# zhaoyizhou1123/OfflineRL-Kit

Measured on AMD Instinct MI355X. Metric: gradient-steps/sec (CQL, batch=256), higher is better.
Workload: dtype f32 storage / accumulate; products on split-fp16 MFMA (every operand = fp16 hi + fp16 lo plane = 22 significand bits, power-of-two operand scales folded back into the fp32 accumulators, hi*hi + hi*lo + lo*hi on v_mfma_f32_16x16x32_f16; the reference's fp32 has 24): losses and Q-values meet the 1e-4

## Files before the change

offlinerl-kit_amd/csrc/engine.h:

```cpp
#pragma once
#include <hip/hip_runtime.h>

#include <map>
#include <set>
#include <string>
#include <vector>

#include "../../include/orl_engine.h"
#include "gemm.h"
#include "kernels.h"
#include "ws_gemm.h"
#include "small_fwd.h"
#include "small_bwd.h"

namespace orl {

void set_error(const std::string& msg);
int fail(const std::string& msg);
#define ORL_HIP(expr)                                                                            \
  do {                                                                                           \
    hipError_t _e = (expr);                                                                      \
    if (_e != hipSuccess) {                                                                      \
      ::orl::set_error(std::string(#expr) + ": " + hipGetErrorString(_e));                       \
      return -1;                                                                                 \
// ... 205 lines not shown
    prof_begin(p3 ? (std::string(tag) + "@p3").c_str() : tag, flops, bytes);
    const hipError_t err = launch();
    prof_end();
    return err == hipSuccess ? 0 : fail(std::string(what) + " launch " + tag + ": " + hipGetErrorString(err));
  }
  int tail_add(const ZOut& out, long out_sm, const ZOut& part, int nparts, int M, int nz1, const char* tag);
  WsFwdP ws_fwd_p(const Mat& X, int M, const NetRef& nr, int layer, const Mat& Y, const Mat* dmask) const;
  int ws_dgrad(const DY& dy, int M, const NetRef& nr, int layer, const Mat& maskH, const Mat* w0_X, const Mat* dX, int max_blocks, const char* tag, int* slabs);
  int ws_wgrad(const DY& dy, const Mat& X, int M, const NetRef& nr, int layer, const Mat* recompute_X0, const char* tag, int* slabs);
  SmallFwdP small_fwd_p(const Mat& X, int M, const NetRef& nr, const Mat* H0, const Mat* H1, const Mat& out) const;
  int linear_fwd(const Mat& X, int M, const NetRef& nr, int layer, const Mat& Y, int epi, const Mat* maskH, const char* tag,
                 int in_row0 = 0, int in_rows = -1, const Mat* tail_out = nullptr, bool* tail_fused = nullptr,
                 const Mat* fuse_X0 = nullptr, const char* tag0 = nullptr, const float* x_dscale = nullptr);
  int tq_scratch_nets = 2;
  int linear_dgrad(const DY& dy, int M, const NetRef& nr, int layer, int col0, int ncols, const Mat* maskH, const Mat& dX, const char* tag,
                   const Mat* w0_X = nullptr, bool store_dx = true, int* w0_slabs = nullptr);
  int linear_wgrad(const DY& dy, const Mat& X, int M, const NetRef& nr, int layer, int ksplit, int slab0, bool with_bias,
                   const char* tag, int in_row0 = 0, int in_rows = -1, bool* fuse_tail = nullptr, int* slabs_out = nullptr,
                   const float* x_dscale = nullptr, const Mat* recompute_X0 = nullptr);
  bool recompute_h0 = false;
  bool recompute_h0_ok(const NetLayout& l, int layer, int M, int nz) const {
    return recompute_h0 && layer == 1 && l.L >= 3 && !l.ens && ws_precision_ok() && ws_wgrad_rows_ok(M, nz);
  }
  int adam(int net, int nnets, int lr_slot, const std::vector<std::pair<long, int>>& segs, int target_net, unsigned long long t_div = 1);
  int polyak(int target_net, int src_net, int nnets);
  void prof_begin(const char* name, double flops, double bytes = 0);
  void prof_end();
  int assemble(const Mat& obs, const Mat* act, const Mat& X, int row0, int rows, int rep);
  int mlp_forward(const Mat& X, int M, const NetRef& nr, std::vector<Mat>& hs, const Mat& out, const char* tag,
                  const SampleJob* jobs = nullptr, int njobs = 0, bool* jobs_done = nullptr);
  int mlp_qgrad(const Mat& X, int M, const NetRef& nr, const Mat& q, const Mat& G, int gc0, int gn, const char* tag, bool* done);
  int mlp_forward_only(const Mat& X, int M, const NetRef& nr, std::vector<Mat>& hs, const Mat& out, const char* tag,
                       const SampleJob* jobs = nullptr, int njobs = 0, bool* jobs_done = nullptr);
  bool fwd_only = false;
  int mlp_forward_dropout(const Mat& X, int M, const NetRef& nr, std::vector<Mat>& hs, const Mat& out, const char* tag, float p,
                          const std::vector<Mat>& masks);
  int scale_inplace(const Mat& m, int rows, int cols, int nets, float s, const Mat* mask, const char* tag);
  bool no_ws = false;
  float bwd_scale = 1.0f;

  int enqueue_sample();
  int enqueue_noise();
  int enqueue_step(int variant);
  int step_variant() const;
  int n_variants() const;
  int build_common();
// ... 12 lines not shown
```

offlinerl-kit_amd/csrc/engine.hip:

```cpp
#include "engine.h"

#include <math.h>
#include <stdio.h>
#include <stdlib.h>
#include <string.h>

#include <algorithm>
#include <tuple>

namespace orl {

static thread_local std::string g_err;
void set_error(const std::string& msg) { g_err = msg; }
int fail(const std::string& msg) {
  set_error(msg);
  return -1;
}

static inline int rup(int x, int m) { return (x + m - 1) / m * m; }

static void add_tensor(NetLayout& l, const std::string& name, long off, std::initializer_list<long> shape) {
  TensorInfo t;
  t.name = name;
  t.off = off;
// ... 431 lines not shown
    }
  }
  const int nz = R * nr.nz1;
  int cfg = pick_cfg(p.M, p.N, p.K, nz);
  if (cfg == CFG_SQ) cfg = CFG_SQ8;
  if (epi == E_BIAS_RELU && ws_precision_ok() && !no_ws && !force_scalar && in_row0 == 0 && in_rows == in &&
      Y.bits && Y.pitch == out && (long)M * nz >= ws_fwd_min_rows) {
    WsFwdP w = ws_fwd_p(X, M, nr, layer, Y, nullptr);
    const bool want_tail = tail_out && tail_fused && layer == l.L - 1 && l.out_dim == 1;
    if (want_tail) { w.tw = nr.w(l.L); w.tb = nr.b(l.L); w.tq = tail_out->zo(); w.tq_sm = tail_out->pitch; }
    const bool elide = want_tail && layer >= 1 && (fwd_only || (elide_top && !l.ens && ws_wgrad_rows_ok(M, nz)));
    if (elide) w.Y.p = nullptr;
    const bool ws_ok = ws_fwd_supported(w, in, out);
    bool fused0 = false;
    if (ws_ok && fuse_X0 && layer == 1 && X.bits && X.pitch == in) {
      w.X0 = fuse_X0->z(); w.x0_pitch = fuse_X0->pitch; w.in0 = l.layer_in(0);
      w.W0 = nr.w(0);
      if (l.ens) { w.w0_sn = 1; w.w0_sk = l.layer_out(0); } else { w.w0_sn = l.layer_in(0); w.w0_sk = 1; }
      w.b0 = nr.b(0);
      w.mb0 = X.zbits(); w.mb0_g = X.bg;
      fused0 = ws_fwd01_supported(w) && aligned16(fuse_X0->p);
      if (!fused0) w.X0.p = nullptr;
      else if (fwd_only || (!want_tail && recompute_h0_ok(l, layer, M, nz))) w.x0_discard = 1;
    }
    if (fuse_X0 && !fused0) {
      if (linear_fwd(*fuse_X0, M, nr, 0, X, E_BIAS_RELU, nullptr, tag0 ? tag0 : tag)) return -1;
      fuse_X0 = nullptr;
    }
    if (ws_ok) {
      bool fwd3 = false;
      if (p3(1) && (fused0 || !w.X0.p) && ws_dump && (!want_tail || ws.count("tq_scratch"))) {
        bool room = true;
        if (want_tail) {
          const Mat& sc = ws.at("tq_scratch");
          room = (long)M <= sc.cs && nr.nz1 <= tq_scratch_nets;
          if (room) w.tq2 = sc.zo();
        }
        if (room) {
          w.np3 = 1; w.dump = ws_dump;
          fwd3 = ws_fwd3_supported(w, in, out);
          if (!fwd3) { w.np3 = 0; w.tq2.p = nullptr; w.dump = nullptr; }
        }
      }
      const double f0 = fused0 ? 2.0 * M * (double)in * (w.in0 + 1) * nz : 0.0;
      if (fused0) bits_live.insert(X.bits);
      if (w.x0_discard) vals_dead.insert(X.p);
// ... 87 lines not shown
  GemmP p;
  memset(&p, 0, sizeof(p));
  p.a_dscale = cur_gscale; p.b_scale = ORL_WSCALE;
  if (mm_prec() == P_SPLIT3) p.a_scale = ORL_GSCALE3;
  p.A = dy.m.z();
  p.a_sr = dy.m.pitch; p.a_sk = 1;
  if (dy.rank1) {
    p.a_trans = 0;
    p.rowv = dy.rowv.z();
    p.colv = nr.w(l.L);
  }
  p.B = nr.w(layer);
  if (l.ens) { p.B.p += (long)col0 * out; p.b_sr = out; p.b_sk = 1; }
  else { p.B.p += col0; p.b_sr = 1; p.b_sk = in; p.b_rlim = (in - col0) & ~3; }
  p.C = dX.p; p.c_s0 = dX.rs; p.c_s1 = dX.cs; p.c_sr = dX.pitch; p.c_sn = 1;
  p.M = M; p.N = ncols; p.K = out;
  p.nz1 = nr.nz1; p.ksplit = 1;
  if (maskH) { p.aux = maskH->z(); p.aux_sr = maskH->pitch; }
  const int nz = R * nr.nz1;
  if (w0_slabs) *w0_slabs = 0;
  if (maskH && maskH->bits && bits_live.count(maskH->bits) && ncols == maskH->pitch && aligned16(maskH->p) && (maskH->pitch & 3) == 0) {
    p.aux_bits = maskH->bits; p.xb_s0 = maskH->brs; p.xb_s1 = maskH->bcs; p.xb_g = maskH->bg;
  }
  if (w0_X && w0_slabs && !store_dx && maskH && dy.rank1 && layer == 1 && col0 == 0 && !l.ens && !force_scalar &&
      ws_precision_ok() && p.aux_bits && dy.m.bits && bits_live.count(dy.m.bits) && out == dy.m.pitch &&
      ncols == in && (long)M * nz >= ws_bwd_min_rows) {
    const int rc = ws_dgrad(dy, M, nr, layer, *maskH, w0_X, nullptr, max_slab, tag, w0_slabs);
    if (rc <= 0) return rc;
  }
  if (!(w0_X && w0_slabs) && maskH && dy.rank1 && col0 == 0 && !force_scalar && ws_precision_ok() && p.aux_bits &&
      dy.m.bits && bits_live.count(dy.m.bits) && out == dy.m.pitch && ncols == in && dX.pitch >= in && (long)M * nz >= ws_bwd_min_rows) {
    const int rc = ws_dgrad(dy, M, nr, layer, *maskH, nullptr, &dX, 1 << 20, tag, nullptr);
    if (rc <= 0) return rc;
  }
  if (w0_X && w0_slabs && !store_dx && maskH && !dy.rank1 && layer == 1 && col0 == 0 && !force_scalar && ws_precision_ok() &&
      p.aux_bits && dy.m.pitch == out && ncols == in && (long)M * nz >= ws_dgrad_plain_min_rows) {
    const int rc = ws_dgrad(dy, M, nr, layer, *maskH, w0_X, nullptr, max_slab, tag, w0_slabs);
    if (rc <= 0) return rc;
  }
  if (w0_X && w0_slabs && maskH && layer == 1 && col0 == 0 && !l.ens && !force_scalar) {
    const int slabs = w0_fused_slabs(p, nz, l.layer_in(0), w0_X->pitch, w0_X->p, w0_X->rs, w0_X->cs, max_slab);
    if (slabs > 0) {
      float* g = grads + nr.g_off;
      p.w0_x = w0_X->z(); p.w0_xsr = w0_X->pitch; p.w0_in = l.layer_in(0);
      p.w0_out = g + l.w_off[0]; p.w0_bias = g + l.b_off[0];
      p.w0_s0 = (long)max_slab * P_train; p.w0_s1 = l.w_ms[0]; p.w0_bs1 = l.b_ms[0]; p.w0_ks = P_train; p.w0_sr = l.layer_in(0);
// ... 47 lines not shown
  if (Krows >= 4096) ks = std::max(ks, wgrad_long_min);
  if (cfg == CFG_SQ && Krows < 1024 && kchunks >= 8) ks = std::max(ks, wgrad_small_ks);
  ks = std::max(1, std::min(ks, std::min(ksplit_cap, kchunks)));
  while (ks > 1 && (kchunks + ks - 1) / ks < 2) --ks;
  return ks;
}

int Engine::ws_wgrad(const DY& dy, const Mat& X, int M, const NetRef& nr, int layer, const Mat* recompute_X0, const char* tag, int* slabs) {
  const NetLayout& l = *nr.lay;
  const int in = l.layer_in(layer), out = l.layer_out(layer), nz = R * nr.nz1;
  const bool derived = dy.rank1 && vals_dead.count(dy.m.p) > 0;
  float* g = grads + nr.g_off;
  WsWgradP w;
  memset(&w, 0, sizeof(w));
  w.H0 = X.z(); w.h0_pitch = X.pitch;
  w.dW = g + l.w_off[layer]; w.db = g + l.b_off[layer];
  w.o_rs = (long)max_slab * P_train; w.o_msw = l.w_ms[layer]; w.o_msb = l.b_ms[layer]; w.o_ks = P_train;
  if (dy.rank1) {
    w.abits = dy.m.zbits(); w.ab_g = dy.m.bg;
    w.dq = dy.rowv.z(); w.dq_sm = dy.rowv.pitch;
    w.wt = nr.w(l.L);
    if (derived) { w.W1 = nr.w(layer); w.b1 = nr.b(layer); }
    else { w.H1 = dy.m.z(); w.h1_pitch = dy.m.pitch; }
    w.dwt = g + l.w_off[l.L]; w.dbt = g + l.b_off[l.L]; w.o_mswt = l.w_ms[l.L]; w.o_msbt = l.b_ms[l.L];
    w.np3 = p3(4) && derived;
    w.lab_clk = lab_clk(72);
  } else {
    w.dZ = dy.m.z(); w.dz_pitch = dy.m.pitch;
    if (recompute_X0) {
      w.X0 = recompute_X0->z(); w.x0_pitch = recompute_X0->pitch; w.in0 = l.layer_in(0);
      w.W0 = nr.w(0); w.w0_sn = l.layer_in(0); w.w0_sk = 1;
      w.b0 = nr.b(0);
    }
  }
  w.M = M; w.nz1 = nr.nz1; w.f32 = ws_f32(); w.gscale = cur_gscale;
  if (!ws_wgrad_supported(w, out, in)) return 1;
  const bool w3 = !dy.rank1 && p3(4) && ws_wgrad3p_supported(w, out, in);
  const int per_z = ws_dgrad_blocks(M, w3 ? 2 * nz : nz, dy.rank1 ? ws_wgrad_slab_cap : max_slab, ws_geo, 1 << 20);
  const double flops = 2.0 * M * (double)in * (dy.rank1 ? out + 2 : out + 1 + (recompute_X0 ? w.in0 + 1 : 0)) * nz;
  const double bytes = dy.rank1 ? nz * ((derived ? M * (double)out / 8 : 4.0 * M * (double)out) + 4.0 * M * (in + 1) + 4.0 * per_z * out * (in + 2))
                                : nz * (4.0 * M * (double)((recompute_X0 ? w.x0_pitch : in) + out) + 4.0 * per_z * out * (in + 1));
  if (timed("ws_wgrad", tag, w3 || w.np3, flops, bytes, [&] { return w3 ? launch_ws_wgrad3p(w, nz, per_z, stream) : launch_ws_wgrad(w, nz, per_z, stream); })) return -1;
  *slabs = per_z;
  return 0;
}

int Engine::linear_wgrad(const DY& dy, const Mat& X, int M, const NetRef& nr, int layer, int ksplit, int slab0, bool with_bias,
                         const char* tag, int in_row0, int in_rows, bool* fuse_tail, int* slabs_out, const float* x_dscale, const Mat* recompute_X0) {
  const NetLayout& l = *nr.lay;
  const int in = l.layer_in(layer), out = l.layer_out(layer);
  if (in_rows < 0) in_rows = in;
  if (slab0 + ksplit > max_slab) return fail("wgrad: slab budget exceeded");
  const bool x_dead = vals_dead.count(X.p) > 0;
  if (x_dead && !(recompute_X0 && layer == 1)) return fail(std::string("wgrad ") + tag + ": the input activation was not stored by the forward pass");
  GemmP p;
  memset(&p, 0, sizeof(p));
  p.a_dscale = cur_gscale; p.b_dscale = x_dscale;
  if (mm_prec() == P_SPLIT3) { p.a_scale = ORL_GSCALE3; if (x_dscale) p.b_scale = ORL_GSCALE3; }
  p.A = dy.m.z();
  p.a_sr = 1; p.a_sk = dy.m.pitch;
  if (out == 1 && dy.m.pitch == 1 && !dy.rank1) p.a_sr = 4;
  if (dy.rank1) {
    p.a_trans = 1;
    p.rowv = dy.rowv.z();
    p.colv = nr.w(l.L);
  }
  p.B = X.z();
  p.b_sr = 1; p.b_sk = X.pitch;
  p.a_rlim = dy.m.pitch & ~3; p.b_rlim = X.pitch & ~3;
  p.ones_row = 1 << 30;
  p.M = out; p.N = in_rows; p.K = M;
  p.nz1 = nr.nz1; p.ksplit = ksplit;
  const long g_rs = (long)max_slab * P_train;
  float* g = grads + nr.g_off + (long)slab0 * P_train;
  if (l.ens) { p.C = g + l.w_off[layer] + (long)in_row0 * out; p.c_sr = 1; p.c_sn = out; }
  else { p.C = g + l.w_off[layer] + in_row0; p.c_sr = in; p.c_sn = 1; }
  p.c_s0 = g_rs; p.c_s1 = l.w_ms[layer]; p.c_ks = P_train;
  if (with_bias) { p.bias_out = g + l.b_off[layer]; p.bo_s0 = g_rs; p.bo_s1 = l.b_ms[layer]; p.bo_ks = P_train; }
  const int nz = R * nr.nz1;
  if (slabs_out) *slabs_out = ksplit;
  if (slabs_out && fuse_tail && dy.rank1 && with_bias && slab0 == 0 && ws_precision_ok() && !force_scalar && !l.ens &&
      dy.m.bits && bits_live.count(dy.m.bits) && out == dy.m.pitch && in_row0 == 0 && in_rows == in && X.pitch == in &&
      ws_wgrad_rows_ok(M, nz)) {
    const int rc = ws_wgrad(dy, X, M, nr, layer, nullptr, tag, slabs_out);
    if (rc == 0) *fuse_tail = true;
    if (rc <= 0) return rc;
  }
  if (slabs_out && !dy.rank1 && with_bias && slab0 == 0 && ws_precision_ok() && !force_scalar && !l.ens && !x_dscale && in_row0 == 0 &&
      in_rows == in && X.pitch == in && dy.m.pitch == out && ws_wgrad_rows_ok(M, nz)) {
    const int rc = ws_wgrad(dy, X, M, nr, layer, x_dead ? recompute_X0 : nullptr, tag, slabs_out);
    if (rc <= 0) return rc;
  }
  if (x_dead) return fail(std::string("wgrad ") + tag + ": the input activation was not stored and the recomputing kernel does not serve this shape");
  if (dy.rank1 && vals_dead.count(dy.m.p)) return fail(std::string("wgrad ") + tag + ": the activation values were not stored by the forward pass");
  if (fuse_tail) {
    *fuse_tail = dy.rank1 && rank1_wgrad_is_fast(p, force_scalar);
    if (*fuse_tail) {
      p.tail_w_out = g + l.w_off[l.L]; p.tail_b_out = g + l.b_off[l.L];
      p.tw_s0 = g_rs; p.tw_s1 = l.w_ms[l.L]; p.tb_s1 = l.b_ms[l.L];
    }
  }
  if (dy.rank1) return run_gemm<PA_RANK1, PB_PLAIN, E_WGRAD>(this, CFG_AUTO, p, nz, tag);
  return run_gemm<PA_PLAIN, PB_PLAIN, E_WGRAD>(this, CFG_AUTO, p, nz, tag);
}

int Engine::adam(int net, int nnets, int lr_slot, const std::vector<std::pair<long, int>>& segs, int target_net, unsigned long long t_div) {
  AdamP a;
// ... 276 lines not shown
      {"ORL_WS_WGRAD_MIN", &ws_wgrad_min_rows, POS_L},
      {"ORL_WS_WGRAD_MIN_M", &ws_wgrad_min_m, POS_I},
      {"ORL_WS_WGRAD_SLABS", &ws_wgrad_slab_cap, POS_I},
      {"ORL_SMALL_FWD", &small_fwd_on, FLAG},
      {"ORL_SMALL_FWD_MAX", &small_fwd_max_rows, POS_L},
      {"ORL_FUSE_SMALL", &fuse_small, FLAG},
      {"ORL_P3", &p3_mask, ANY_I},
      {"ORL_WGRAD_WG_TARGET", &wgrad_wg_target, POS_I},
      {"ORL_WGRAD_LONG_MIN", &wgrad_long_min, POS_I},
      {"ORL_WGRAD_SMALL_KS", &wgrad_small_ks, POS_I},
  };
  for (const auto& k : knobs) {
    const char* f = getenv(k.name);
    if (!f) continue;
    const long v = atol(f);
    switch (k.kind) {
      case FLAG: *(bool*)k.field = v != 0; break;
      case NFLAG: *(bool*)k.field = v == 0; break;
      case POS_I: if (v > 0) *(int*)k.field = (int)v; break;
      case POS_L: if (v > 0) *(long*)k.field = v; break;
      case ANY_I: *(int*)k.field = (int)v; break;
    }
  }
  ws_wgrad_slab_cap = std::min(ws_wgrad_slab_cap, max_slab);
  if (cus >= 8 && cus <= 256) ws_geo.cus = cus;
}

int Engine::init(const orl_config& c) {
  cfg = c;
  int ndev = 0;
  if (hipGetDeviceCount(&ndev) != hipSuccess || ndev == 0) return fail("no HIP device available: the update engine needs an MI355X (gfx950)");
  if (c.device < 0 || c.device >= ndev) return fail("bad device ordinal");
  dev = c.device;
  ORL_HIP(hipSetDevice(dev));
  if (c.precision < 0 || c.precision > 2) return fail("precision must be 0 (fp32 MFMA), 1 (split-precision MFMA: two fp16 planes) or 2 (three fp16 planes where a kernel has them, fp32 MFMA elsewhere)");
  if (c.actor_dropout != 0.f && (c.algo != ORL_ALGO_IQL || !(c.actor_dropout > 0.f && c.actor_dropout < 1.f)))
    return fail("actor_dropout: supported for IQL only (run_iql.py --dropout_rate), 0 < p < 1");
  if (build_layouts(c, lay, net_off, net_is_target, &P_train, &P_tgt)) return -1;
  ORL_HIP(hipStreamCreateWithFlags(&stream, hipStreamNonBlocking));
  ORL_HIP(hipStreamCreateWithFlags(&side_stream, hipStreamNonBlocking));
  ORL_HIP(hipEventCreateWithFlags(&ev_fork, hipEventDisableTiming));
  ORL_HIP(hipEventCreateWithFlags(&ev_join, hipEventDisableTiming));
  ws_geo.one_round = c.ws_one_round != 0;
  ws_geo.cus = (c.ws_cus >= 8 && c.ws_cus <= 256) ? c.ws_cus : 256;
  read_env();
  R = c.n_runs; B = c.batch_size; od = c.obs_dim; ad = c.act_dim;
// ... 1238 lines not shown
```

offlinerl-kit_amd/csrc/ws_gemm.h:

```cpp
#pragma once
#include <hip/hip_runtime.h>
#include <cstdlib>
#include <stdint.h>

#include "gemm.h"

namespace orl {

#ifdef SB_LAB_CLOCK
#define WS_STAMP(i) do { if (p.lab_clk && threadIdx.x == 0 && blockIdx.x == 0 && blockIdx.z == 0) p.lab_clk[i] = __builtin_amdgcn_s_memtime(); } while (0)
#else
#define WS_STAMP(i) do { } while (0)
#endif

struct WsFwdP {
  ZPtr X; int x_pitch;
  ZPtr W;
  long w_sn, w_sk;
  ZPtr bias;
  ZOut Y; int y_pitch;
  ZBits mb; int mb_g;
  ZPtr tw;
  ZPtr tb;
  ZOut tq; long tq_sm;
// ... 134 lines not shown
  ZPtr X0; int x0_pitch, in0;
  ZPtr W0; long w0_sn, w0_sk;
  ZPtr b0;
  unsigned long long* lab_clk;
  int M, nz1, groups;
  int f32;
  int np3;
  const float* gscale;
};
enum { WW_IMG = WS_ROWS * WS_K };
static constexpr size_t ws_wgrad_lds_bytes(bool plain = false, bool recompute = false, bool p3 = false) {
  return (size_t)2 * ((plain || p3) ? 4 : 3) * WW_IMG * 2 + (size_t)2 * (p3 ? 3 : 2) * WS_ROWS * 16 * 2 + (recompute ? sizeof(float) * 2 * WS_ROWS * WS_XLP : 0);
}

static inline bool ws_wgrad_supported(const WsWgradP& p, int K, int N) {
  if (p.dZ.p) {
    if (K != WS_K || N != WS_N || p.M < 256 || (p.M % WS_ROWS)) return false;
    if (!p.dZ.vec4() || (p.dz_pitch & 3)) return false;
    if (p.X0.p) return p.W0.p && p.b0.p && p.in0 + 1 <= 32 && p.in0 < p.x0_pitch + 1 && p.x0_pitch <= 32 && p.in0 <= p.x0_pitch && WS_ROWS * p.x0_pitch <= 2 * WS_NT;
    return p.H0.vec4() && !(p.h0_pitch & 3);
  }
  if (K != WS_K || N != WS_N || p.M < 256 || (p.M % WS_ROWS) || !p.abits.p || p.ab_g != 8) return false;
  if (p.np3 && (p.H1.p || !p.W1.p)) return false;
  if (!p.H0.vec4() || (p.h0_pitch & 3)) return false;
  if (!p.H1.p && p.W1.p && (!p.b1.p || !p.dwt || !p.dbt)) return false;
  if (p.H1.p && (!p.H1.vec4() || (p.h1_pitch & 3) || !p.dwt || !p.dbt)) return false;
  return p.wt.vec4();
}
hipError_t launch_ws_wgrad(WsWgradP p, int nz, int per_z, hipStream_t st);
static constexpr size_t ws_wgrad3p_lds_bytes() { return (size_t)2 * (3 * WS_ROWS * 128 + 3 * WS_ROWS * WS_K) * 2 + (size_t)WS_ROWS * 16 * 2; }
static inline bool ws_wgrad3p_supported(const WsWgradP& p, int K, int N) {
  return p.dZ.p && !p.X0.p && ws_wgrad_supported(p, K, N);
}
hipError_t launch_ws_wgrad3p(WsWgradP p, int nz, int per_z, hipStream_t st);

}
```

offlinerl-kit_amd/csrc/ws_wgrad.hip:

```cpp
#include "ws_device.h"

namespace orl {

__device__ inline int ww_off(int r, int chunk, int half) { return r * WS_K + ((chunk ^ (2 * (r & 7))) << 3) + (half << 2); }

__device__ inline s16x4 ww_tr(const hx_t* img, int row0, int col0, int lane) {
  const int li = lane & 15, lq = lane >> 4, row = row0 + 4 * lq + (li >> 2), col = col0 + 4 * (li & 3);
  const hx_t* a = img + ww_off(row, col >> 3, (col >> 2) & 1);
  return __builtin_amdgcn_ds_read_tr16_b64_v4i16((s16x4 __attribute__((address_space(3)))*)a);
}

template <int MODE>
__device__ __forceinline__ void ww_finish(const WsWgradP& p, float* ws_smem, const f32x4 (&acc)[16][2], const f32x4 (&accb)[2], const f32x4& tacc,
                                          const f32x4& bacc, float dqsum, const float* __restrict__ wtg, int z0, int z1, int ncol0, float inv = 1.0f) {
  constexpr bool TAILS = (MODE == 1);
  const int tid = threadIdx.x, wave = tid >> 6, lane = tid & 63, li = lane & 15, lq = lane >> 4;
  const long so = z0 * p.o_rs + (long)blockIdx.x * p.o_ks;
  float* dW = p.dW + so + z1 * p.o_msw;
  float* db = p.db + so + z1 * p.o_msb;
  if (MODE == 2) {
    const float* __restrict__ W1g = p.W1.p + z0 * p.W1.s0 + z1 * p.W1.s1;
    float* red = ws_smem;
#pragma unroll
    for (int kb2 = 0; kb2 < 16; kb2 += 2) {
// ... 85 lines not shown
  float* red = ws_smem;
  *(f32x4*)&red[(tid >> 6) * WS_K + 4 * (tid & 63)] = tacc;
  *(f32x4*)&red[(8 + (tid >> 6)) * WS_K + 4 * (tid & 63)] = bacc;
  if ((tid & 63) == 0) red[16 * WS_K + (tid >> 6)] = dqsum;
  __syncthreads();
  if (tid < WS_K) {
    float a = 0.f, b = 0.f;
#pragma unroll
    for (int w = 0; w < 8; ++w) { a += red[w * WS_K + tid]; b += red[(8 + w) * WS_K + tid]; }
    p.dwt[so + z1 * p.o_mswt + tid] = a;
    db[tid] = wtg[tid] * b;
  }
  if (tid == 0) {
    float a = 0.f;
#pragma unroll
    for (int w = 0; w < 8; ++w) a += red[16 * WS_K + w];
    p.dbt[so + z1 * p.o_msbt] = a;
  }
}

template <int MODE>
__global__ __launch_bounds__(WS_NT) void ws_wgrad_kernel(const WsWgradP p) {
  static_assert(WS_NW == 8 && WS_ROWS == 32, "8 waves x 32 columns, 32-row groups");
  constexpr bool TAILS = (MODE == 1), PLAIN = (MODE == 3 || MODE == 4), RECOMP = (MODE == 4), P3 = (MODE == 5);
  constexpr int NPL = (PLAIN || P3) ? 4 : 3;
  constexpr int DQP = P3 ? 3 : 2;
  extern __shared__ __attribute__((aligned(16))) float ws_smem[];
  hx_t* img = (hx_t*)ws_smem;
  __shared__ u32x2_t mlut[16];
  const int tid = threadIdx.x, wave = tid >> 6, lane = tid & 63, li = lane & 15, lq = lane >> 4;
  const int z = blockIdx.z, z0 = z / p.nz1, z1 = z - z0 * p.nz1;
  const unsigned int* __restrict__ ab = PLAIN ? nullptr : p.abits.p + z0 * p.abits.s0 + z1 * p.abits.s1;
  const float* __restrict__ dqg = PLAIN ? nullptr : p.dq.p + z0 * p.dq.s0 + z1 * p.dq.s1;
  const float* __restrict__ H0g = p.H0.p + z0 * p.H0.s0 + z1 * p.H0.s1;
  const float* __restrict__ wtg = PLAIN ? nullptr : p.wt.p + z0 * p.wt.s0 + z1 * p.wt.s1;
  const int ncol0 = 32 * wave;
  const float gsc = p.gscale ? p.gscale[z0] : 1.f;

  WS_STAMP(0);
  f32x4 acc[16][2], accb[2];
#pragma unroll
  for (int kb = 0; kb < 16; ++kb)
#pragma unroll
    for (int nb = 0; nb < 2; ++nb) acc[kb][nb] = (f32x4){0.f, 0.f, 0.f, 0.f};
  accb[0] = accb[1] = (f32x4){0.f, 0.f, 0.f, 0.f};

  f32x4 s0[4];
// ... 33 lines not shown
#pragma unroll
  for (int i = 0; i < 2; ++i) {
    const int e = tid + WS_NT * i;
    xr[i] = RECOMP ? e / (RECOMP ? p.x0_pitch : 1) : 0; xc[i] = RECOMP ? e - xr[i] * p.x0_pitch : 0;
    if (RECOMP && e >= xe) { xr[i] = 0; xc[i] = 32; }
  }
  auto loadX = [&](int g) __attribute__((always_inline)) {
#pragma unroll
    for (int i = 0; i < 2; ++i) { const int e = tid + WS_NT * i; sx[i] = X0g[(long)g * xe + (e < xe ? e : xe - 1)]; }
  };
  auto storeX = [&](int xbuf) __attribute__((always_inline)) {
#pragma unroll
    for (int i = 0; i < 2; ++i) {
      const float x = (xc[i] == p.in0) ? 1.0f : sx[i];
      hx_t* row = (hx_t*)(Xl + (xbuf * WS_ROWS + xr[i]) * WS_XLP);
      const bool pad = xc[i] >= 32;
      hx_t hh, ll;
      orl_split1(x, hh, ll);
      row[pad ? 64 : xc[i]] = hh;
      row[pad ? 65 : 32 + xc[i]] = ll;
    }
  };
  hx8 xah, xal;
  auto prod_x = [&](int xbuf, int s) __attribute__((always_inline)) {
    const hx_t* xrow = (const hx_t*)(Xl + (xbuf * WS_ROWS + 16 * s + li) * WS_XLP) + 8 * lq;
    xah = *(const hx8*)xrow; xal = *(const hx8*)(xrow + 32);
  };
  auto prod_block = [&](int buf, int s, int cb) __attribute__((always_inline)) {
    hx_t* gh = img + (long)buf * NPL * WW_IMG + (NPL - 2) * WW_IMG;
    hx_t* gl = gh + WW_IMG;
    f32x4 v = (f32x4){0.f, 0.f, 0.f, 0.f};
    v = ORL_MFMA_16x16x32(b0l[cb], xah, v);
    v = ORL_MFMA_16x16x32(b0h[cb], xal, v);
    v = ORL_MFMA_16x16x32(b0h[cb], xah, v);
    orl_relu_mask4(v);
    hx4 h, l;
    orl_split4(v, h, l);
    const int k = ncol0 + 16 * cb + 4 * lq;
    const int o = ww_off(16 * s + li, k >> 3, (k >> 2) & 1);
    *(hx4*)(gh + o) = h;
    *(hx4*)(gl + o) = l;
  };
  const unsigned int vo_h0 = (unsigned int)((tid >> 6) * p.h0_pitch + 4 * (tid & 63));
  const unsigned int vo_h1 = (TAILS || PLAIN) ? (unsigned int)((tid >> 6) * h1_pitch + 4 * (tid & 63)) : 0u;
  const unsigned int vo_dq = (unsigned int)((tid >> 6) * (int)p.dq_sm);
  const unsigned int vo_ab = (unsigned int)((tid >> 4) * p.ab_g + ((tid & 15) >> 1));
  auto load_piece = [&](int g, int i) __attribute__((always_inline)) {
    const long row0 = (long)g * WS_ROWS + 8 * i;
    if (!RECOMP) s0[i] = *(const f32x4*)&(H0g + row0 * p.h0_pitch)[vo_h0];
    if (TAILS || PLAIN) s1[i] = *(const f32x4*)&(H1g + row0 * h1_pitch)[vo_h1];
    if (!PLAIN) sdq[i] = (dqg + row0 * p.dq_sm)[vo_dq];
  };
  auto load_mask = [&](int g) __attribute__((always_inline)) {
    if (!PLAIN) sm_word = (ab + (long)g * WS_ROWS * p.ab_g)[vo_ab];
  };
  auto load_group = [&](int g) __attribute__((always_inline)) {
    load_mask(g);
#pragma unroll
// ... 26 lines not shown
      hx_t* zh = img + (long)buf * NPL * WW_IMG;
      orl_split4(s1[i] * gsc, h, l);
      *(hx4*)(zh + o) = h;
      *(hx4*)(zh + WW_IMG + o) = l;
      return;
    }
    const float dqs = sdq[i] * gsc;
    if (P3) {
      hx4 m;
      hx_t* g3 = img + (long)buf * NPL * WW_IMG + WW_IMG;
      orl_split4x3(s0[i] * dqs, h, m, l);
      *(hx4*)(g3 + o) = h;
      *(hx4*)(g3 + WW_IMG + o) = m;
      *(hx4*)(g3 + 2 * WW_IMG + o) = l;
      if (kq == 0) {
        hx_t hh, mm, ll;
        orl_split1x3(dqs, hh, mm, ll);
        hx_t* dqi = dqimg + (long)buf * DQP * WS_ROWS * 16;
        dqi[r * 16] = hh; dqi[WS_ROWS * 16 + r * 16] = mm; dqi[2 * WS_ROWS * 16 + r * 16] = ll;
        dqsum += sdq[i];
      }
      return;
    }
    orl_split4(s0[i] * dqs, h, l);
    *(hx4*)(gh + o) = h;
    *(hx4*)(gl + o) = l;
    if (TAILS) {
#pragma unroll
      for (int j = 0; j < 4; ++j) { tacc[j] += sdq[i] * s1[i][j]; bacc[j] += s1[i][j] > 0.f ? sdq[i] : 0.f; }
      dqsum += sdq[i];
    } else if (kq == 0) {
      hx_t hh, ll;
      orl_split1(dqs, hh, ll);
      hx_t* dqi = dqimg + (long)buf * 2 * WS_ROWS * 16;
      dqi[r * 16] = hh; dqi[WS_ROWS * 16 + r * 16] = ll;
      if (MODE == 2) dqsum += sdq[i];
    }
  };
  auto store_group = [&](int buf) __attribute__((always_inline)) {
    store_mask(buf);
#pragma unroll
    for (int i = 0; i < 4; ++i) store_piece(buf, i);
  };
  if (!TAILS) for (int e = tid; e < 2 * DQP * WS_ROWS * 16 / 2; e += WS_NT) ((unsigned int*)dqimg)[e] = 0u;
  if (PLAIN) {
    __syncthreads();
    if (tid < 2 * WS_ROWS) (dqimg + (long)(tid >> 5) * 2 * WS_ROWS * 16)[(tid & 31) * 16] = (hx_t)1.0f;
  }
  if (tid < 16) mlut[tid] = (u32x2_t){((tid & 1u) | ((tid & 2u) << 15)) * ORL_HX_ONE_BITS, (((tid >> 2) & 1u) | ((tid & 8u) << 13)) * ORL_HX_ONE_BITS};
  if (RECOMP) for (int e = tid; e < 2 * WS_ROWS * WS_XLP; e += WS_NT) Xl[e] = 0.f;
  __syncthreads();

  const int g0 = blockIdx.x, gs = gridDim.x;
  WS_STAMP(1);
  if (RECOMP && g0 < p.groups) {
    loadX(g0);
    storeX(0);
    if (g0 + gs < p.groups) loadX(g0 + gs);
    __syncthreads();
#pragma unroll
    for (int s = 0; s < 2; ++s) {
      prod_x(0, s);
#pragma unroll
      for (int cb = 0; cb < 2; ++cb) prod_block(0, s, cb);
    }
    if (g0 + gs < p.groups) storeX(1);
  }
  if (g0 < p.groups) {
    load_group(g0);
    store_group(0);
    if (g0 + gs < p.groups) load_group(g0 + gs);
  }
  __syncthreads();
  auto iteration = [&](int g, int it, bool steady) __attribute__((always_inline)) {
    const int buf = it & 1;
    const bool more = steady || g + gs < p.groups, more2 = steady || g + 2 * gs < p.groups;
    const hx_t* mi = img + (long)buf * NPL * WW_IMG;
    const hx_t* ml = mi + WW_IMG;
    const hx_t* gh = mi + (P3 ? 1 : NPL - 2) * WW_IMG;
    const hx_t* gl = gh + (P3 ? 2 : 1) * WW_IMG;
    const hx_t* gm = gh + WW_IMG;
    const hx_t* dqi = dqimg + (long)buf * DQP * WS_ROWS * 16;
    {
      auto cat = [](s16x4 x, s16x4 y) __attribute__((always_inline)) {
        hx8 r;
        *(s16x4*)&r = x; *((s16x4*)&r + 1) = y;
        return r;
      };
      hx8 bh[2], bl[2], bm[2];
#pragma unroll
      for (int nb = 0; nb < 2; ++nb) {
        bh[nb] = cat(ww_tr(gh, 0, ncol0 + 16 * nb, lane), ww_tr(gh, 16, ncol0 + 16 * nb, lane));
        bl[nb] = cat(ww_tr(gl, 0, ncol0 + 16 * nb, lane), ww_tr(gl, 16, ncol0 + 16 * nb, lane));
        if (P3) bm[nb] = cat(ww_tr(gm, 0, ncol0 + 16 * nb, lane), ww_tr(gm, 16, ncol0 + 16 * nb, lane));
// ... 42 lines not shown
            accb[0] = ORL_MFMA_16x16x32(e0, bdh, accb[0]);
            accb[1] = ORL_MFMA_16x16x32(e1, bdh, accb[1]);
          } else {
            accb[0] = ORL_MFMA_16x16x32(c0, bdl, accb[0]);
            accb[1] = ORL_MFMA_16x16x32(c1, bdl, accb[1]);
            if (P3) {
              accb[0] = ORL_MFMA_16x16x32(c0, bdm, accb[0]);
              accb[1] = ORL_MFMA_16x16x32(c1, bdm, accb[1]);
            }
          }
          accb[0] = ORL_MFMA_16x16x32(c0, bdh, accb[0]);
          accb[1] = ORL_MFMA_16x16x32(c1, bdh, accb[1]);
        }
        if (kp < 4) {
          if (more) store_piece(buf ^ 1, kp);
          if (more2) load_piece(g + 2 * gs, kp);
        }
        if (RECOMP) {
          if (kp == 0 && more2) loadX(g + 2 * gs);
          if (kp >= 4 && more) {
            if (!(kp & 1)) prod_x(buf ^ 1, (kp - 4) >> 1);
            prod_block(buf ^ 1, (kp - 4) >> 1, kp & 1);
          }
          if (kp == 7 && more2) storeX(buf);
        }
        if (kp == 5) {
          if (more) store_mask(buf ^ 1);
          if (more2) load_mask(g + 2 * gs);
        }
      }
    }
    __syncthreads();
  };
  int g = g0, it = 0;
  WS_STAMP(2);
  for (; MODE != 1 && g + 2 * gs < p.groups; g += gs, ++it) iteration(g, it, true);
  for (; g < p.groups; g += gs, ++it) iteration(g, it, false);
  WS_STAMP(3);

  ww_finish<(MODE == 4 ? 3 : (MODE == 5 ? 2 : MODE))>(p, ws_smem, acc, accb, tacc, bacc, dqsum, wtg, z0, z1, ncol0, 1.0f / gsc);
  WS_STAMP(4);
}

enum { WW32_P = 272, WW32_IMG = WS_ROWS * WW32_P };
static constexpr size_t ws_wgrad32_lds_bytes(bool recompute = false) {
  return sizeof(float) * ((size_t)2 * 2 * WW32_IMG + 2 * WS_ROWS + (recompute ? 2 * WS_ROWS * WS_XLP : 0)) > sizeof(float) * 17 * WS_K
             ? sizeof(float) * ((size_t)2 * 2 * WW32_IMG + 2 * WS_ROWS + (recompute ? 2 * WS_ROWS * WS_XLP : 0)) : sizeof(float) * 17 * WS_K;
}

template <int MODE>
__global__ __launch_bounds__(WS_NT) void ws_wgrad32_kernel(const WsWgradP p) {
  static_assert(WS_NW == 8 && WS_ROWS == 32, "8 waves x 32 columns, 32-row groups");
  constexpr bool TAILS = (MODE == 1), PLAIN = (MODE == 3 || MODE == 4), RECOMP = (MODE == 4);
  extern __shared__ __attribute__((aligned(16))) float ws_smem[];
  float* img = ws_smem;
  float* dqs = img + 2 * 2 * WW32_IMG;
  float* Xl = dqs + 2 * WS_ROWS;
  __shared__ f32x4 mlut[16];
  const int tid = threadIdx.x, wave = tid >> 6, lane = tid & 63, li = lane & 15, lq = lane >> 4;
  const int z = blockIdx.z, z0 = z / p.nz1, z1 = z - z0 * p.nz1;
  const unsigned int* __restrict__ ab = PLAIN ? nullptr : p.abits.p + z0 * p.abits.s0 + z1 * p.abits.s1;
  const float* __restrict__ dqg = PLAIN ? nullptr : p.dq.p + z0 * p.dq.s0 + z1 * p.dq.s1;
  const float* __restrict__ H0g = p.H0.p + z0 * p.H0.s0 + z1 * p.H0.s1;
// ... 194 lines not shown
    }
    __syncthreads();
  };
  int g = g0, it = 0;
  for (; MODE != 1 && g + 2 * gs < p.groups; g += gs, ++it) iteration(g, it, true);
  for (; g < p.groups; g += gs, ++it) iteration(g, it, false);
  ww_finish<(MODE == 4 ? 3 : MODE)>(p, ws_smem, acc, accb, tacc, bacc, dqsum, wtg, z0, z1, ncol0);
}

hipError_t launch_ws_wgrad(WsWgradP p, int nz, int per_z, hipStream_t st) {
  p.groups = p.M / WS_ROWS;
  static const hipError_t attr_err = [] {
    hipError_t e = hipFuncSetAttribute((const void*)ws_wgrad_kernel<0>, hipFuncAttributeMaxDynamicSharedMemorySize, (int)ws_wgrad_lds_bytes());
    if (e == hipSuccess) e = hipFuncSetAttribute((const void*)ws_wgrad_kernel<1>, hipFuncAttributeMaxDynamicSharedMemorySize, (int)ws_wgrad_lds_bytes());
    if (e == hipSuccess) e = hipFuncSetAttribute((const void*)ws_wgrad_kernel<2>, hipFuncAttributeMaxDynamicSharedMemorySize, (int)ws_wgrad_lds_bytes());
    if (e == hipSuccess) e = hipFuncSetAttribute((const void*)ws_wgrad32_kernel<0>, hipFuncAttributeMaxDynamicSharedMemorySize, (int)ws_wgrad32_lds_bytes());
    if (e == hipSuccess) e = hipFuncSetAttribute((const void*)ws_wgrad32_kernel<1>, hipFuncAttributeMaxDynamicSharedMemorySize, (int)ws_wgrad32_lds_bytes());
    if (e == hipSuccess) e = hipFuncSetAttribute((const void*)ws_wgrad32_kernel<2>, hipFuncAttributeMaxDynamicSharedMemorySize, (int)ws_wgrad32_lds_bytes());
    if (e == hipSuccess) e = hipFuncSetAttribute((const void*)ws_wgrad_kernel<3>, hipFuncAttributeMaxDynamicSharedMemorySize, (int)ws_wgrad_lds_bytes(true));
    if (e == hipSuccess) e = hipFuncSetAttribute((const void*)ws_wgrad32_kernel<3>, hipFuncAttributeMaxDynamicSharedMemorySize, (int)ws_wgrad32_lds_bytes());
    if (e == hipSuccess) e = hipFuncSetAttribute((const void*)ws_wgrad_kernel<4>, hipFuncAttributeMaxDynamicSharedMemorySize, (int)ws_wgrad_lds_bytes(true, true));
    if (e == hipSuccess) e = hipFuncSetAttribute((const void*)ws_wgrad32_kernel<4>, hipFuncAttributeMaxDynamicSharedMemorySize, (int)ws_wgrad32_lds_bytes(true));
    if (e == hipSuccess) e = hipFuncSetAttribute((const void*)ws_wgrad_kernel<5>, hipFuncAttributeMaxDynamicSharedMemorySize, (int)ws_wgrad_lds_bytes(false, false, true));
    return e;
  }();
  if (attr_err != hipSuccess) return attr_err;
  const dim3 grid(per_z, 1, nz), block(WS_NT);
  if (p.dZ.p && p.X0.p) {
    if (p.f32) hipLaunchKernelGGL(ws_wgrad32_kernel<4>, grid, block, ws_wgrad32_lds_bytes(true), st, p);
    else hipLaunchKernelGGL(ws_wgrad_kernel<4>, grid, block, ws_wgrad_lds_bytes(true, true), st, p);
    return hipGetLastError();
  }
  if (p.dZ.p) {
    if (p.f32) hipLaunchKernelGGL(ws_wgrad32_kernel<3>, grid, block, ws_wgrad32_lds_bytes(), st, p);
    else hipLaunchKernelGGL(ws_wgrad_kernel<3>, grid, block, ws_wgrad_lds_bytes(true), st, p);
    return hipGetLastError();
  }
  if (p.np3) {
    hipLaunchKernelGGL(ws_wgrad_kernel<5>, grid, block, ws_wgrad_lds_bytes(false, false, true), st, p);
    return hipGetLastError();
  }
  if (p.f32) {
    if (p.H1.p) hipLaunchKernelGGL(ws_wgrad32_kernel<1>, grid, block, ws_wgrad32_lds_bytes(), st, p);
    else if (p.W1.p) hipLaunchKernelGGL(ws_wgrad32_kernel<2>, grid, block, ws_wgrad32_lds_bytes(), st, p);
    else hipLaunchKernelGGL(ws_wgrad32_kernel<0>, grid, block, ws_wgrad32_lds_bytes(), st, p);
    return hipGetLastError();
  }
  if (p.H1.p) hipLaunchKernelGGL(ws_wgrad_kernel<1>, grid, block, ws_wgrad_lds_bytes(), st, p);
  else if (p.W1.p) hipLaunchKernelGGL(ws_wgrad_kernel<2>, grid, block, ws_wgrad_lds_bytes(), st, p);
  else hipLaunchKernelGGL(ws_wgrad_kernel<0>, grid, block, ws_wgrad_lds_bytes(), st, p);
  return hipGetLastError();
}

}
```

Baseline: 53260.

## Recompute first hidden layer in fused top-layer wgrad instead of storing it

New measurement: 55160, median of 6. +3.6%, better.

```diff
diff --git a/offlinerl-kit_amd/csrc/engine.h b/offlinerl-kit_amd/csrc/engine.h
--- a/offlinerl-kit_amd/csrc/engine.h
+++ b/offlinerl-kit_amd/csrc/engine.h
@@ -251,6 +251,11 @@
   bool recompute_h0_ok(const NetLayout& l, int layer, int M, int nz) const {
     return recompute_h0 && layer == 1 && l.L >= 3 && !l.ens && ws_precision_ok() && ws_wgrad_rows_ok(M, nz);
   }
+  bool recompute_h0_top = true;
+  bool recompute_h0_top_ok(const NetLayout& l, int layer, int M, int nz, bool top_elided) const {
+    return recompute_h0_top && layer == 1 && l.L == 2 && l.out_dim == 1 && !l.ens && top_elided && !fwd_only && cfg.precision == 1 && use_ws &&
+           !force_scalar && ws_wgrad_rows_ok(M, nz) && (M % WS_ROWS) == 0;
+  }
   int adam(int net, int nnets, int lr_slot, const std::vector<std::pair<long, int>>& segs, int target_net, unsigned long long t_div = 1);
   int polyak(int target_net, int src_net, int nnets);
   void prof_begin(const char* name, double flops, double bytes = 0);
diff --git a/offlinerl-kit_amd/csrc/engine.hip b/offlinerl-kit_amd/csrc/engine.hip
--- a/offlinerl-kit_amd/csrc/engine.hip
+++ b/offlinerl-kit_amd/csrc/engine.hip
@@ -477,6 +477,7 @@
       fused0 = ws_fwd01_supported(w) && aligned16(fuse_X0->p);
       if (!fused0) w.X0.p = nullptr;
       else if (fwd_only || (!want_tail && recompute_h0_ok(l, layer, M, nz))) w.x0_discard = 1;
+      else if (want_tail && recompute_h0_top_ok(l, layer, M, nz, elide) && Y.bg == 8) w.x0_discard = 1;
     }
     if (fuse_X0 && !fused0) {
       if (linear_fwd(*fuse_X0, M, nr, 0, X, E_BIAS_RELU, nullptr, tag0 ? tag0 : tag)) return -1;
@@ -610,6 +611,7 @@
   if (maskH && maskH->bits && bits_live.count(maskH->bits) && ncols == maskH->pitch && aligned16(maskH->p) && (maskH->pitch & 3) == 0) {
     p.aux_bits = maskH->bits; p.xb_s0 = maskH->brs; p.xb_s1 = maskH->bcs; p.xb_g = maskH->bg;
   }
+  if (maskH && !p.aux_bits && vals_dead.count(maskH->p)) return fail(std::string("dgrad ") + tag + ": the masking activation was not stored by the forward pass and its mask bits do not serve this shape");
   if (w0_X && w0_slabs && !store_dx && maskH && dy.rank1 && layer == 1 && col0 == 0 && !l.ens && !force_scalar &&
       ws_precision_ok() && p.aux_bits && dy.m.bits && bits_live.count(dy.m.bits) && out == dy.m.pitch &&
       ncols == in && (long)M * nz >= ws_bwd_min_rows) {
@@ -703,6 +705,12 @@
     w.wt = nr.w(l.L);
     if (derived) { w.W1 = nr.w(layer); w.b1 = nr.b(layer); }
     else { w.H1 = dy.m.z(); w.h1_pitch = dy.m.pitch; }
+    if (recompute_X0) {
+      if (!derived) return 1;
+      w.X0 = recompute_X0->z(); w.x0_pitch = recompute_X0->pitch; w.in0 = l.layer_in(0);
+      w.W0 = nr.w(0); w.w0_sn = l.layer_in(0); w.w0_sk = 1;
+      w.b0 = nr.b(0);
+    }
     w.dwt = g + l.w_off[l.L]; w.dbt = g + l.b_off[l.L]; w.o_mswt = l.w_ms[l.L]; w.o_msbt = l.b_ms[l.L];
     w.np3 = p3(4) && derived;
     w.lab_clk = lab_clk(72);
@@ -718,8 +726,8 @@
   if (!ws_wgrad_supported(w, out, in)) return 1;
   const bool w3 = !dy.rank1 && p3(4) && ws_wgrad3p_supported(w, out, in);
   const int per_z = ws_dgrad_blocks(M, w3 ? 2 * nz : nz, dy.rank1 ? ws_wgrad_slab_cap : max_slab, ws_geo, 1 << 20);
-  const double flops = 2.0 * M * (double)in * (dy.rank1 ? out + 2 : out + 1 + (recompute_X0 ? w.in0 + 1 : 0)) * nz;
-  const double bytes = dy.rank1 ? nz * ((derived ? M * (double)out / 8 : 4.0 * M * (double)out) + 4.0 * M * (in + 1) + 4.0 * per_z * out * (in + 2))
+  const double flops = 2.0 * M * (double)in * ((dy.rank1 ? out + 2 : out + 1) + (recompute_X0 ? w.in0 + 1 : 0)) * nz;
+  const double bytes = dy.rank1 ? nz * ((derived ? M * (double)out / 8 : 4.0 * M * (double)out) + 4.0 * M * ((recompute_X0 ? w.x0_pitch : in) + 1) + 4.0 * per_z * out * (in + 2))
                                 : nz * (4.0 * M * (double)((recompute_X0 ? w.x0_pitch : in) + out) + 4.0 * per_z * out * (in + 1));
   if (timed("ws_wgrad", tag, w3 || w.np3, flops, bytes, [&] { return w3 ? launch_ws_wgrad3p(w, nz, per_z, stream) : launch_ws_wgrad(w, nz, per_z, stream); })) return -1;
   *slabs = per_z;
@@ -763,7 +771,7 @@
   if (slabs_out && fuse_tail && dy.rank1 && with_bias && slab0 == 0 && ws_precision_ok() && !force_scalar && !l.ens &&
       dy.m.bits && bits_live.count(dy.m.bits) && out == dy.m.pitch && in_row0 == 0 && in_rows == in && X.pitch == in &&
       ws_wgrad_rows_ok(M, nz)) {
-    const int rc = ws_wgrad(dy, X, M, nr, layer, nullptr, tag, slabs_out);
+    const int rc = ws_wgrad(dy, X, M, nr, layer, x_dead ? recompute_X0 : nullptr, tag, slabs_out);
     if (rc == 0) *fuse_tail = true;
     if (rc <= 0) return rc;
   }
@@ -1086,6 +1094,7 @@
       case ANY_I: *(int*)k.field = (int)v; break;
     }
   }
+  if (getenv("ORL_WS_RECOMPUTE_H0")) recompute_h0_top = recompute_h0;
   ws_wgrad_slab_cap = std::min(ws_wgrad_slab_cap, max_slab);
   if (cus >= 8 && cus <= 256) ws_geo.cus = cus;
 }
diff --git a/offlinerl-kit_amd/csrc/ws_gemm.h b/offlinerl-kit_amd/csrc/ws_gemm.h
--- a/offlinerl-kit_amd/csrc/ws_gemm.h
+++ b/offlinerl-kit_amd/csrc/ws_gemm.h
@@ -180,6 +180,8 @@
   }
   if (K != WS_K || N != WS_N || p.M < 256 || (p.M % WS_ROWS) || !p.abits.p || p.ab_g != 8) return false;
   if (p.np3 && (p.H1.p || !p.W1.p)) return false;
+  if (p.X0.p && (p.np3 || p.f32 || p.H1.p || !p.W1.p || !p.W0.p || !p.b0.p || p.in0 + 1 > 32 || p.in0 > p.x0_pitch || p.x0_pitch > 32 ||
+                 WS_ROWS * p.x0_pitch > 2 * WS_NT)) return false;
   if (!p.H0.vec4() || (p.h0_pitch & 3)) return false;
   if (!p.H1.p && p.W1.p && (!p.b1.p || !p.dwt || !p.dbt)) return false;
   if (p.H1.p && (!p.H1.vec4() || (p.h1_pitch & 3) || !p.dwt || !p.dbt)) return false;
diff --git a/offlinerl-kit_amd/csrc/ws_wgrad.hip b/offlinerl-kit_amd/csrc/ws_wgrad.hip
--- a/offlinerl-kit_amd/csrc/ws_wgrad.hip
+++ b/offlinerl-kit_amd/csrc/ws_wgrad.hip
@@ -131,7 +131,9 @@
 template <int MODE>
 __global__ __launch_bounds__(WS_NT) void ws_wgrad_kernel(const WsWgradP p) {
   static_assert(WS_NW == 8 && WS_ROWS == 32, "8 waves x 32 columns, 32-row groups");
-  constexpr bool TAILS = (MODE == 1), PLAIN = (MODE == 3 || MODE == 4), RECOMP = (MODE == 4), P3 = (MODE == 5);
+  constexpr bool TAILS = (MODE == 1), PLAIN = (MODE == 3 || MODE == 4), RTOP = (MODE == 6), RECOMP = (MODE == 4 || RTOP), P3 = (MODE == 5);
+  constexpr bool DERIVED = (MODE == 2 || RTOP);
+  constexpr int WS_XDQ = 34;
   constexpr int NPL = (PLAIN || P3) ? 4 : 3;
   constexpr int DQP = P3 ? 3 : 2;
   extern __shared__ __attribute__((aligned(16))) float ws_smem[];
@@ -211,9 +213,17 @@
     }
   };
   hx8 xah, xal;
+  float xdq = 0.f;
   auto prod_x = [&](int xbuf, int s) __attribute__((always_inline)) {
     const hx_t* xrow = (const hx_t*)(Xl + (xbuf * WS_ROWS + 16 * s + li) * WS_XLP) + 8 * lq;
     xah = *(const hx8*)xrow; xal = *(const hx8*)(xrow + 32);
+    if (RTOP) xdq = Xl[(xbuf * WS_ROWS + 16 * s + li) * WS_XLP + WS_XDQ];
+  };
+  auto storeDQ = [&](int xbuf) __attribute__((always_inline)) {
+    if (lane == 0) {
+#pragma unroll
+      for (int i = 0; i < 4; ++i) Xl[(xbuf * WS_ROWS + 8 * i + wave) * WS_XLP + WS_XDQ] = sdq[i] * gsc;
+    }
   };
   auto prod_block = [&](int buf, int s, int cb) __attribute__((always_inline)) {
     hx_t* gh = img + (long)buf * NPL * WW_IMG + (NPL - 2) * WW_IMG;
@@ -223,6 +233,10 @@
     v = ORL_MFMA_16x16x32(b0h[cb], xal, v);
     v = ORL_MFMA_16x16x32(b0h[cb], xah, v);
     orl_relu_mask4(v);
+    if (RTOP) {
+#pragma unroll
+      for (int j = 0; j < 4; ++j) v[j] = v[j] * xdq;
+    }
     hx4 h, l;
     orl_split4(v, h, l);
     const int k = ncol0 + 16 * cb + 4 * lq;
@@ -295,9 +309,11 @@
       }
       return;
     }
-    orl_split4(s0[i] * dqs, h, l);
-    *(hx4*)(gh + o) = h;
-    *(hx4*)(gl + o) = l;
+    if (!RTOP) {
+      orl_split4(s0[i] * dqs, h, l);
+      *(hx4*)(gh + o) = h;
+      *(hx4*)(gl + o) = l;
+    }
     if (TAILS) {
 #pragma unroll
       for (int j = 0; j < 4; ++j) { tacc[j] += sdq[i] * s1[i][j]; bacc[j] += s1[i][j] > 0.f ? sdq[i] : 0.f; }
@@ -307,7 +323,7 @@
       orl_split1(dqs, hh, ll);
       hx_t* dqi = dqimg + (long)buf * 2 * WS_ROWS * 16;
       dqi[r * 16] = hh; dqi[WS_ROWS * 16 + r * 16] = ll;
-      if (MODE == 2) dqsum += sdq[i];
+      if (DERIVED) dqsum += sdq[i];
     }
   };
   auto store_group = [&](int buf) __attribute__((always_inline)) {
@@ -326,23 +342,43 @@
 
   const int g0 = blockIdx.x, gs = gridDim.x;
   WS_STAMP(1);
-  if (RECOMP && g0 < p.groups) {
-    loadX(g0);
-    storeX(0);
-    if (g0 + gs < p.groups) loadX(g0 + gs);
-    __syncthreads();
-#pragma unroll
-    for (int s = 0; s < 2; ++s) {
-      prod_x(0, s);
-#pragma unroll
-      for (int cb = 0; cb < 2; ++cb) prod_block(0, s, cb);
-    }
-    if (g0 + gs < p.groups) storeX(1);
-  }
-  if (g0 < p.groups) {
-    load_group(g0);
-    store_group(0);
-    if (g0 + gs < p.groups) load_group(g0 + gs);
+  if (RTOP) {
+    if (g0 < p.groups) {
+      const bool nxt = g0 + gs < p.groups;
+      load_group(g0);
+      loadX(g0);
+      storeX(0);
+      storeDQ(0);
+      store_group(0);
+      if (nxt) { load_group(g0 + gs); loadX(g0 + gs); }
+      __syncthreads();
+#pragma unroll
+      for (int s = 0; s < 2; ++s) {
+        prod_x(0, s);
+#pragma unroll
+        for (int cb = 0; cb < 2; ++cb) prod_block(0, s, cb);
+      }
+      if (nxt) { storeX(1); storeDQ(1); }
+    }
+  } else {
+    if (RECOMP && g0 < p.groups) {
+      loadX(g0);
+      storeX(0);
+      if (g0 + gs < p.groups) loadX(g0 + gs);
+      __syncthreads();
+#pragma unroll
+      for (int s = 0; s < 2; ++s) {
+        prod_x(0, s);
+#pragma unroll
+        for (int cb = 0; cb < 2; ++cb) prod_block(0, s, cb);
+      }
+      if (g0 + gs < p.groups) storeX(1);
+    }
+    if (g0 < p.groups) {
+      load_group(g0);
+      store_group(0);
+      if (g0 + gs < p.groups) load_group(g0 + gs);
+    }
   }
   __syncthreads();
   auto iteration = [&](int g, int it, bool steady) __attribute__((always_inline)) {
@@ -431,7 +467,7 @@
             if (!(kp & 1)) prod_x(buf ^ 1, (kp - 4) >> 1);
             prod_block(buf ^ 1, (kp - 4) >> 1, kp & 1);
           }
-          if (kp == 7 && more2) storeX(buf);
+          if (kp == 7 && more2) { storeX(buf); if (RTOP) storeDQ(buf); }
         }
         if (kp == 5) {
           if (more) store_mask(buf ^ 1);
@@ -447,7 +483,7 @@
   for (; g < p.groups; g += gs, ++it) iteration(g, it, false);
   WS_STAMP(3);
 
-  ww_finish<(MODE == 4 ? 3 : (MODE == 5 ? 2 : MODE))>(p, ws_smem, acc, accb, tacc, bacc, dqsum, wtg, z0, z1, ncol0, 1.0f / gsc);
+  ww_finish<(MODE == 4 ? 3 : ((MODE == 5 || MODE == 6) ? 2 : MODE))>(p, ws_smem, acc, accb, tacc, bacc, dqsum, wtg, z0, z1, ncol0, 1.0f / gsc);
   WS_STAMP(4);
 }
 
@@ -688,6 +724,7 @@
     if (e == hipSuccess) e = hipFuncSetAttribute((const void*)ws_wgrad_kernel<4>, hipFuncAttributeMaxDynamicSharedMemorySize, (int)ws_wgrad_lds_bytes(true, true));
     if (e == hipSuccess) e = hipFuncSetAttribute((const void*)ws_wgrad32_kernel<4>, hipFuncAttributeMaxDynamicSharedMemorySize, (int)ws_wgrad32_lds_bytes(true));
     if (e == hipSuccess) e = hipFuncSetAttribute((const void*)ws_wgrad_kernel<5>, hipFuncAttributeMaxDynamicSharedMemorySize, (int)ws_wgrad_lds_bytes(false, false, true));
+    if (e == hipSuccess) e = hipFuncSetAttribute((const void*)ws_wgrad_kernel<6>, hipFuncAttributeMaxDynamicSharedMemorySize, (int)ws_wgrad_lds_bytes(false, true));
     return e;
   }();
   if (attr_err != hipSuccess) return attr_err;
@@ -702,6 +739,10 @@
     else hipLaunchKernelGGL(ws_wgrad_kernel<3>, grid, block, ws_wgrad_lds_bytes(true), st, p);
     return hipGetLastError();
   }
+  if (p.X0.p) {
+    hipLaunchKernelGGL(ws_wgrad_kernel<6>, grid, block, ws_wgrad_lds_bytes(false, true), st, p);
+    return hipGetLastError();
+  }
   if (p.np3) {
     hipLaunchKernelGGL(ws_wgrad_kernel<5>, grid, block, ws_wgrad_lds_bytes(false, false, true), st, p);
     return hipGetLastError();
```
